# SaumikDana/Bayesian-Markov-chain-Monte-Carlo

Hardware: AMD Instinct MI355X
Metric: ode_steps_x_chains_per_sec (higher is better)
Workload: dtype f64

## Files before the change

### bayesian-markov-chain-monte-carlo_amd/csrc/rsf_device.h

```cpp
#pragma once
#include <hip/hip_runtime.h>
#include <stdint.h>

#include <type_traits>

#include "rsf_math.h"

namespace rsf {

struct Consts {
  double mu_ref, V_ref, k1, mu0;
  double a_def, b_def;
  double h, hh, h6;
  double inv_dt;
  double t0, dt;
  double inv_vref;
  double cacc;
  const double *vl;
  const double *data;
  int64_t group_chains;
  int32_t nout;
  int32_t S;
  int32_t kc;
  int32_t nchunks;
  double vl_lo, vl_hi;
};

__device__ __forceinline__ void select_group(Consts &K) {
  if (K.group_chains > 0) K.data += ((int64_t)blockIdx.x * blockDim.x / K.group_chains) * K.nout;
}

struct Lane {
  double inv_dc;
  double vdc;
  double kprime;
  double kia;
  double khh, kh, kh6;
  double vk;
  double beta;
  double kvk;
  double vrw;
  double hhdw, hdw;
  double cv;
  double h6v;
  double boa;
  double nhboa;
  double tc;
  double hhd, hd, h6d;
  double bh;
  double c_l1p, c_l1q;
  double c_em1;
  double cv2;
  double boa2;
  double bh2, bh4;
};

template <int T>
__device__ __forceinline__ void set_tier(Lane &L);

template <bool DAMP>
__device__ __forceinline__ Lane make_lane(double dc, double a, double b, const Consts &K) {
  Lane L;
  const double inv_a = fm::rcp(a);
  L.inv_dc = fm::rcp(dc);
  L.kprime = (1e-2 * 10) * L.inv_dc;
  L.kia = L.kprime * inv_a;
  L.khh = L.kia * K.hh;
  L.kh = L.kia * K.h;
  L.kh6 = L.kia * K.h6;
  const double via = K.V_ref * inv_a;
  L.vdc = K.V_ref * L.inv_dc;
  L.vk = via * L.kprime;
  L.beta = (b * K.V_ref) * (1.0 / (1e-2 * 10));
  L.kvk = K.k1 * via;
  const double ikw = DAMP ? fm::rcp(L.kvk) : 1.0;
  const double vkw = DAMP ? L.vk * ikw : L.vk;
  L.cv = K.cacc * vkw;
  L.h6v = K.h6 * vkw;
  L.boa = b * inv_a;
  L.tc = -K.mu_ref * inv_a;
  L.hhd = K.hh * L.vdc;
  L.hd = K.h * L.vdc;
  L.h6d = K.h6 * L.vdc;
  L.vrw = DAMP ? K.V_ref * ikw : K.V_ref;
  L.hhdw = DAMP ? L.hhd * ikw : L.hhd;
  L.hdw = DAMP ? L.hd * ikw : L.hd;
  L.nhboa = -0.5 * L.boa;
  L.bh = L.beta * fm::rcp(L.hhd);
  L.cv2 = 2.0 * L.cv;
  L.boa2 = 2.0 * L.boa;
  L.bh2 = -2.0 * L.bh;
  L.bh4 = 4.0 * L.bh;
  set_tier<2>(L);
  return L;
}


struct State {
  double ms, x, V;
  double w, rx;
};

template <bool DAMP>
__device__ __forceinline__ void rhs_tail(double w, double rx, double x, double vl, const Lane &L,
                                         const Consts &K, double &d0, double &d1, double &d2) {
  d1 = __builtin_fma(-w, x, 1.0);
  d0 = __builtin_fma(-K.V_ref, w, vl);
  const double bt = (L.beta * d1) * rx;
  double g = d0 - bt;
  if (DAMP) {
    const double kw = L.kvk * w;
    d0 = __builtin_fma(-kw, g, d0);
    g = d0 - bt;
    d2 = kw * g;
  } else {
    d2 = w * g;
  }
}

__device__ __forceinline__ void eval_full(double ms, double x, const Lane &L, const Consts &K, double &w, double &rx) {
  w = fm::exp(__builtin_fma(-L.boa, fm::log(x), __builtin_fma(ms, L.kia, L.tc)));
  rx = fm::rcp(x);
}

enum Tier : int { TIGHT = 0, NARROW = 1, WIDE = 2, FULL = 3 };

__device__ __forceinline__ double local_value(double x) {
  asm volatile("" : "+v"(x));
  return x;
}

template <bool DAMP, int T>
__device__ __forceinline__ void tier_enter(State &s, const Lane &L) {
  s.rx *= L.hhd;
  if (DAMP) s.w *= L.kvk;
}
template <int T>
__device__ __forceinline__ void tier_x(State &s, const Lane &L) { s.x = L.hhd * fm::rcp(s.rx); }
template <bool DAMP, int T>
__device__ __forceinline__ void tier_leave(State &s, const Lane &L) {
  tier_x<T>(s, L);
  s.rx *= fm::rcp(local_value(L.hhd));
  if (DAMP) s.w *= fm::rcp(local_value(L.kvk));
}
template <bool DAMP, int T>
__device__ __forceinline__ void eval_full_t(State &s, const Lane &L, const Consts &K) {
  eval_full(s.ms, s.x, L, K, s.w, s.rx);
  tier_enter<DAMP, T>(s, L);
}
template <bool DAMP, int T>
__device__ __forceinline__ void resync_t(State &s, const Lane &L, const Consts &K) {
  tier_x<T>(s, L);
  eval_full_t<DAMP, T>(s, L, K);
}


struct Guard {
  float rho, dlt;
  float dlt_h;
  float rho_f;
};

__device__ __forceinline__ float hi_as_float(double x) { return __builtin_bit_cast(float, __double2hiint(x)); }
constexpr float hi_pow2(int e) { return __builtin_bit_cast(float, (1023 + e) << 20); }


template <int T>
__device__ __forceinline__ void set_tier(Lane &L) {
  L.c_l1p = L.boa * (1.0 / 3.0);
  L.c_l1q = L.boa * (-1.0 / 4.0);
  L.c_em1 = T == TIGHT ? 1.0 / 24.0 : (T == NARROW ? 1.0 / 720.0 : 1.0 / 40320.0);
  asm volatile("" : "+v"(L.c_l1p), "+v"(L.c_l1q), "+v"(L.c_em1));
}

template <int T>
__device__ __forceinline__ bool guard_ok(const Guard &g) {
  return (g.rho < (T == WIDE ? hi_pow2(-11) : (T == NARROW ? hi_pow2(-14) : hi_pow2(-20)))) &&
         (g.dlt < (T == TIGHT ? hi_pow2(-9) : (T == NARROW ? hi_pow2(-7) : hi_pow2(-5)))) && (T != TIGHT || g.dlt_h < hi_pow2(-10));
}

constexpr float hi_pow2_34(int e) { return __builtin_bit_cast(float, ((1023 + e - 1) << 20) | 0x80000); }
template <int T>
__device__ __forceinline__ bool calm_enough(const Guard &g) {
  static_assert(T == NARROW || T == WIDE, "TIGHT has no tighter tier");
  return T == WIDE ? (g.rho < hi_pow2_34(-14) && g.dlt < hi_pow2_34(-7))
                   : (g.rho < hi_pow2_34(-20) && g.dlt < hi_pow2_34(-10));
}

constexpr int kResync = 512;

template <bool DAMP>
__device__ __forceinline__ double rk4_cold(State &s, double vl0, double vlm, double vl1, const Lane &L,
                                           const Consts &K) {
  double k0 = 0.0, k1 = 0.0, s0 = 0.0, s1 = 0.0, s2 = 0.0;
#pragma nounroll
  for (int st = 0; st < 4; ++st) {
    const double c = st == 0 ? 0.0 : (st == 3 ? K.h : K.hh);
    const double wgt = (st == 0 || st == 3) ? 1.0 : 2.0;
    const double vl = st == 0 ? vl0 : (st == 3 ? vl1 : vlm);
    const double x1 = __builtin_fma(c * L.vdc, k1, s.x);
    double w, rx, d0, d1, d2;
    eval_full(__builtin_fma(c, k0, s.ms), x1, L, K, w, rx);
    rhs_tail<DAMP>(w, rx, x1, vl, L, K, d0, d1, d2);
    s0 = __builtin_fma(wgt, d0, s0);
    s1 = __builtin_fma(wgt, d1, s1);
    s2 = __builtin_fma(wgt, d2, s2);
    k0 = d0;
    k1 = d1;
  }
  s.ms = __builtin_fma(K.h6, s0, s.ms);
  s.x = __builtin_fma(L.h6d, s1, s.x);
  return s2;
}

template <int T, bool HALF, bool SHORT = false, bool GUARD = true>
__device__ __forceinline__ void tight_incr(double rho, double dk, const Lane &L, double w0, double &w, double &q, Guard &g) {
  static_assert(!SHORT || (T == TIGHT && HALF), "the short series is for TIGHT's half-step stages");
  static_assert(GUARD || T == TIGHT, "only TIGHT has an a-priori bound");
  if constexpr (GUARD) g.rho = __builtin_fmaxf(g.rho, __builtin_fabsf(hi_as_float(rho)));
  double pb = L.nhboa;
  if (T == NARROW) pb = __builtin_fma(rho, L.c_l1p, pb);
  if (T == WIDE) pb = __builtin_fma(rho, __builtin_fma(rho, L.c_l1q, L.c_l1p), pb);
  const double dlt = __builtin_fma(-rho, __builtin_fma(rho, pb, L.boa), dk);
  if constexpr (GUARD) {
    if (T == TIGHT && HALF) g.dlt_h = __builtin_fmaxf(g.dlt_h, __builtin_fabsf(hi_as_float(dlt)));
    else g.dlt = __builtin_fmaxf(g.dlt, __builtin_fabsf(hi_as_float(dlt)));
  }
  double e = SHORT ? 1.0 / 6.0 : L.c_em1;
  if (T == WIDE) {
    e = fm::hfma(e, dlt, 1.0 / 5040.0);
    e = fm::hfma(e, dlt, 1.0 / 720.0);
  }
  if (T != TIGHT) {
    e = fm::hfma(e, dlt, 1.0 / 120.0);
    e = fm::hfma(e, dlt, 1.0 / 24.0);
  }
  if (!SHORT) e = fm::hfma(e, dlt, 1.0 / 6.0);
  e = __builtin_fma(e, dlt, 0.5);
  e = __builtin_fma(e, dlt, 1.0);
  w = __builtin_fma(w0 * dlt, e, w0);
  const double r1 = __builtin_fma(rho, rho, -rho);
  q = r1;
  if (T != TIGHT) q = __builtin_fma(-rho, q, -rho);
  if (T == WIDE) q = __builtin_fma(-rho, q, -rho);
}

template <bool GUARD = true>
__device__ __forceinline__ void tight_incr_doubled(double c1, double dk, const Lane &L, double w0, double &w, double &brx, Guard &g) {
  if constexpr (GUARD) g.rho_f = __builtin_fmaxf(g.rho_f, __builtin_fabsf(hi_as_float(c1)));
  const double dlt = __builtin_fma(-c1, __builtin_fma(-c1, L.boa2, L.boa2), dk);
  if constexpr (GUARD) g.dlt = __builtin_fmaxf(g.dlt, __builtin_fabsf(hi_as_float(dlt)));
  double e = fm::hfma(L.c_em1, dlt, 1.0 / 6.0);
  e = __builtin_fma(e, dlt, 0.5);
  e = __builtin_fma(e, dlt, 1.0);
  w = __builtin_fma(w0 * dlt, e, w0);
  brx = __builtin_fma(c1, __builtin_fma(c1, L.bh4, L.bh2), L.bh);
}

template <bool DAMP>
__device__ __forceinline__ void rhs_tight(double w, double xr, double Rh, double vl, double brx, double vr, double &d0, double &d1,
                                          double &g) {
  d1 = __builtin_fma(-w, xr, Rh);
  d0 = __builtin_fma(-vr, w, vl);
  g = __builtin_fma(-brx, d1, d0);
  if (DAMP) {
    d0 = __builtin_fma(-w, g, d0);
    g = __builtin_fma(-w, g, g);
  }
}

template <bool DAMP, int T, bool INSTEP = false, bool GUARD = true>
__device__ __forceinline__ double rk4_tight(State &s, double vl0, double vlm, double vl1, const Lane &L, const Consts &K, Guard &g,
                                            double obs = 0.0, double *ssq = nullptr, bool first = false) {
  static_assert(!INSTEP || T == TIGHT, "the in-step sum of squares is the TIGHT step's");
  static_assert(GUARD || INSTEP, "the unguarded step is the in-step mode's");
  double a0, a1, a2, b0, b1, b2, c0, c1, c2, e0, e1, e2, w, q;
  const double Rh = s.rx;
  const double vr = L.vrw, xh = L.hhdw, xf = L.hdw;
  rhs_tight<DAMP>(s.w, xh, Rh, vl0, L.bh, vr, a0, a1, a2);
  double sv = s.w * a2;
  tight_incr<T, true, INSTEP, GUARD>(a1, L.khh * a0, L, s.w, w, q, g);
  rhs_tight<DAMP>(w, __builtin_fma(xh, a1, xh), Rh, vlm, __builtin_fma(L.bh, q, L.bh), vr, b0, b1, b2);
  double sm = w * b2;
  tight_incr<T, true, INSTEP, GUARD>(b1, L.khh * b0, L, s.w, w, q, g);
  rhs_tight<DAMP>(w, __builtin_fma(xh, b1, xh), Rh, vlm, __builtin_fma(L.bh, q, L.bh), vr, c0, c1, c2);
  sm = __builtin_fma(w, c2, sm);
  if constexpr (INSTEP) {
    double brx;
    tight_incr_doubled<GUARD>(c1, L.kh * c0, L, s.w, w, brx, g);
    rhs_tight<DAMP>(w, __builtin_fma(xf, c1, xh), Rh, vl1, brx, vr, e0, e1, e2);
  } else {
    tight_incr<T, false>(c1 + c1, L.kh * c0, L, s.w, w, q, g);
    rhs_tight<DAMP>(w, __builtin_fma(xf, c1, xh), Rh, vl1, __builtin_fma(L.bh, q, L.bh), vr, e0, e1, e2);
  }
  sv = __builtin_fma(w, e2, sv);
  const double t0 = a0 + 2.0 * b0 + 2.0 * c0 + e0;
  const double t1 = a1 + 2.0 * b1 + 2.0 * c1 + e1;
  const double rho = t1 * (1.0 / 3.0);
  tight_incr<T, false, false, GUARD>(rho, L.kh6 * t0, L, s.w, w, q, g);
  s.ms = __builtin_fma(K.h6, t0, s.ms);
  s.w = w;
  s.rx = __builtin_fma(Rh, q, Rh);
  if constexpr (INSTEP) {
    const double r = __builtin_fma(sv, L.cv, __builtin_fma(sm, L.cv2, -obs));
    *ssq = first ? r * r : __builtin_fma(r, r, *ssq);
    return 0.0;
  }
  return __builtin_fma(2.0, sm, sv);
}

__device__ __forceinline__ State initial_state(double dc, const Lane &L, const Consts &K) {
  State s;
  s.ms = (K.mu0 * dc) * (1.0 / (1e-2 * 10));
  s.x = K.V_ref * ((dc * K.inv_vref) * L.inv_dc);
  s.V = K.V_ref;
  eval_full(s.ms, s.x, L, K, s.w, s.rx);
  return s;
}

constexpr int kLdsPad = 0;
__device__ __forceinline__ int lds_data_offset(const Consts &K) { return 2 * K.S * K.kc + 1 + kLdsPad; }
__device__ __forceinline__ int lds_d0_offset(const Consts &K) { return lds_data_offset(K) + K.kc; }

__device__ __forceinline__ void stage_chunk(double *lds, const Consts &K, int k0, int kn) {
  const int nv = 2 * K.S * kn + 1;
  const int base = 2 * K.S * (k0 - 1);
  __syncthreads();
  for (int i = threadIdx.x; i < nv; i += blockDim.x) lds[i] = K.vl[base + i];
  if (K.data) {
    double *ld = lds + lds_data_offset(K);
    for (int i = threadIdx.x; i < kn; i += blockDim.x) ld[i] = K.data[k0 + i];
    if (threadIdx.x == 0) lds[lds_d0_offset(K)] = K.data[0];
  }
  __syncthreads();
}

struct Emit {
  int ko;
  int phase;
  double vprev;
};

template <bool WANT_SSQ, bool WANT_ACC>
__device__ __forceinline__ void emit_at(double vnow, double vprev, int ko, double obs, const Consts &K, int k0,
                                        double &ssq, bool active, double *acc_out, int64_t stride) {
  const double ak = (vnow - vprev) * K.inv_dt;
  if (WANT_ACC && active) acc_out[(int64_t)(k0 + ko) * stride] = ak;
  if (WANT_SSQ) {
    const double r = ak - obs;
    ssq = __builtin_fma(r, r, ssq);
  }
}

template <bool WANT_SSQ, bool WANT_ACC>
__device__ __forceinline__ void emit_incr(double dvs, int ko, double obs, const Lane &L, int k0, double &ssq,
                                          bool active, double *acc_out, int64_t stride) {
  if (WANT_ACC && active) acc_out[(int64_t)(k0 + ko) * stride] = dvs * L.cv;
  if (WANT_SSQ) {
    const double r = __builtin_fma(dvs, L.cv, -obs);
    ssq = __builtin_fma(r, r, ssq);
  }
}

template <bool WANT_SSQ, bool WANT_ACC>
__device__ __forceinline__ void emit_sample(double vnow, Emit &em, double obs, const Consts &K, int k0, double &ssq,
                                            bool active, double *acc_out, int64_t stride) {
  emit_at<WANT_SSQ, WANT_ACC>(vnow, em.vprev, em.ko, obs, K, k0, ssq, active, acc_out, stride);
  em.vprev = vnow;
  ++em.ko;
}

template <bool DAMP, int T, int NU>
__device__ __forceinline__ bool trip_fast(const double *v, const Lane &L, const Consts &K, State &s, double (&dv)[NU], bool *calm = nullptr) {
  Guard g = {0, 0, 0, 0};
#pragma unroll
  for (int j = 0; j < NU; ++j) dv[j] = rk4_tight<DAMP, T>(s, v[2 * j], v[2 * j + 1], v[2 * j + 2], L, K, g);
  if constexpr (T != TIGHT) {
    if (calm) *calm = calm_enough<T>(g);
  }
  return !guard_ok<T>(g);
}

template <bool DAMP, int T, int NU>
__device__ __forceinline__ void trip_cold(const double *v, const Lane &L, const Consts &K, State &s, double (&dv)[NU]) {
  tier_x<T>(s, L);
#pragma unroll 1
  for (int j = 0; j < NU; ++j) {
    const double r = rk4_cold<DAMP>(s, v[2 * j], v[2 * j + 1], v[2 * j + 2], L, K);
#pragma unroll
    for (int m = 0; m < NU; ++m) dv[m] = m == j ? r : dv[m];
  }
  eval_full_t<DAMP, T>(s, L, K);
}

template <bool DAMP, int T, int NU>
__device__ __forceinline__ void trip_cold_ssq(const double *v, const double *ob, const Lane &L, const Consts &K, State &s, double &ssq) {
  tier_x<T>(s, L);
#pragma unroll 1
  for (int j = 0; j < NU; ++j) {
    const double dvs = rk4_cold<DAMP>(s, v[2 * j], v[2 * j + 1], v[2 * j + 2], L, K);
    emit_incr<true, false>(dvs, j, ob[j], L, 0, ssq, false, nullptr, 0);
  }
  eval_full_t<DAMP, T>(s, L, K);
}

template <bool DAMP, int NU>
__device__ __forceinline__ void trip_cold_plain(const double *v, const Lane &L, const Consts &K, State &s, double (&dv)[NU]) {
#pragma unroll 1
  for (int j = 0; j < NU; ++j) {
    const double r = rk4_cold<DAMP>(s, v[2 * j], v[2 * j + 1], v[2 * j + 2], L, K);
#pragma unroll
    for (int m = 0; m < NU; ++m) dv[m] = m == j ? r : dv[m];
  }
  eval_full(s.ms, s.x, L, K, s.w, s.rx);
}

constexpr int kFullRetry = 32;
constexpr int kCalmSteps = 16;
struct Wave {
  unsigned long long alive;
  unsigned long long need[3];
  unsigned long long stiff;
  int next_resync;
  int full_run;
  int calm;
  uint32_t steps[4], redone, lane_steps;
  double vl_lo, vl_hi;
  unsigned long long never;
  bool guard_next;
  uint32_t unguarded;
};

template <int NU>
struct TightBound {
  static constexpr double R = 0x1.0p-20, B = 0x1.0p-21, Dmax = 0.9 * 0x1.0p-9, gm1 = 1.02 * NU * Dmax;
  static constexpr double G = 1.02 * NU, kap = (NU + 1) * R, Bmax = 0.9 * B;
  static_assert(NU * Dmax < 0.035, "exp(x) - 1 <= 1.02 x needs x < 0.035");
};

__device__ __forceinline__ unsigned long long ballot(bool p) { return __builtin_amdgcn_ballot_w64(p); }
__device__ __forceinline__ bool lane_in(unsigned long long mask) { return (mask >> (threadIdx.x & 63)) & 1; }
template <int CTRL>
__device__ __forceinline__ double dpp_move(double v) {
  const int lo = __builtin_amdgcn_update_dpp(0, __double2loint(v), CTRL, 0xF, 0xF, false);
  const int hi = __builtin_amdgcn_update_dpp(0, __double2hiint(v), CTRL, 0xF, 0xF, false);
  return __hiloint2double(hi, lo);
}

template <int NU>
__device__ __forceinline__ void wave_begin(Wave &W, bool active, const Lane &L, const Consts &K) {
  const double dk = 1.2 * K.V_ref * K.h * L.kia;
  using TB = TightBound<NU>;
  const double dmin = __builtin_fma(__builtin_fabs(L.kh), 0.5 * (K.vl_hi - K.vl_lo), __builtin_fabs(L.boa) * TB::R);
  const double rmin = __builtin_fabs(L.hhd) * __builtin_fma(dmin, TB::G, TB::kap);
  W.never = ballot(active && !(dmin < TB::Dmax && rmin < TB::Bmax));
  W.guard_next = false;
  W.alive = ballot(active);
  W.need[0] = ballot(active && !(dk < 0x1.0p-9));
  W.need[1] = ballot(active && !(dk < 0x1.0p-7));
  W.need[2] = W.stiff = ballot(active && !(dk < 0x1.0p-3));
  W.next_resync = kResync;
  W.full_run = 0;
  W.calm = 0;
  W.vl_lo = K.vl_lo;
  W.vl_hi = K.vl_hi;
  asm volatile("" : "+s"(W.vl_lo), "+s"(W.vl_hi));
}

__device__ __forceinline__ int wave_tier(const Wave &W) {
  return (W.need[2] & W.alive) ? FULL : ((W.need[1] & W.alive) ? WIDE : ((W.need[0] & W.alive) ? NARROW : TIGHT));
}

template <bool DAMP, int NU, bool GUARD = true>
__device__ __forceinline__ unsigned long long trip_fast_ssq(const double *v, const double (&obs)[NU], const Lane &L, const Consts &K, State &s,
                                                            double &tsum) {
  Guard g = {0, 0, 0, 0};
#pragma unroll
  for (int j = 0; j < NU; ++j) rk4_tight<DAMP, TIGHT, true, GUARD>(s, v[2 * j], v[2 * j + 1], v[2 * j + 2], L, K, g, obs[j], &tsum, j == 0);
  if constexpr (!GUARD) return 0ull;
  return ballot(!(g.rho < hi_pow2(-20))) | ballot(!(g.rho_f < hi_pow2(-21))) | ballot(!(g.dlt < hi_pow2(-9))) | ballot(!(g.dlt_h < hi_pow2(-10)));
}

template <bool DAMP, int NU>
__device__ __forceinline__ unsigned long long tight_needs_guard(const State &s, const Lane &L, const Wave &W) {
  using TB = TightBound<NU>;
  constexpr double R = TB::R, B = TB::B, Dmax = TB::Dmax, gm1 = TB::gm1;
  const double p = L.vrw * s.w;
  const double c = __builtin_fma(-s.w, L.hhdw, s.rx);
  double D0 = __builtin_fma(__builtin_fabs(p), gm1, __builtin_fmax(__builtin_fabs(W.vl_hi - p), __builtin_fabs(W.vl_lo - p)));
  if (DAMP) D0 = __builtin_fma((1.0 + gm1) * __builtin_fabs(s.w), __builtin_fma(__builtin_fabs(L.bh), B, D0), D0);
  const double D = __builtin_fma(__builtin_fabs(L.kh), D0, __builtin_fabs(L.boa) * R);
  const double rb = __builtin_fma(__builtin_fabs(s.rx) + __builtin_fabs(c), __builtin_fma(D, TB::G, TB::kap), __builtin_fabs(c));
  return ballot(!(D < Dmax)) | ballot(!(rb < TB::Bmax));
}

template <bool WANT_SSQ, bool WANT_ACC, bool S1, int NU>
__device__ __forceinline__ void emit_trip(const double (&dv)[NU], const double (&obs)[NU], const double *ld, int r, State &s, Emit &em,
                                          const Lane &L, const Consts &K, int k0, double &ssq, bool active, double *acc_out, int64_t stride) {
  if (S1) {
#pragma unroll
    for (int j = 0; j < NU; ++j) emit_incr<WANT_SSQ, WANT_ACC>(dv[j], r + j, obs[j], L, k0, ssq, active, acc_out, stride);
  } else {
#pragma unroll
    for (int j = 0; j < NU; ++j) {
      s.V = __builtin_fma(L.h6v, dv[j], s.V);
      if (++em.phase == K.S) {
        em.phase = 0;
        const double o = WANT_SSQ ? ld[em.ko] : 0.0;
        emit_sample<WANT_SSQ, WANT_ACC>(s.V, em, o, K, k0, ssq, active, acc_out, stride);
      }
    }
  }
}

constexpr int kTightUnroll = 8;
constexpr int kNarrowUnroll = 8, kWiderUnroll = 4;
template <bool DAMP, bool WANT_SSQ, bool WANT_ACC, int T, bool S1, int NU, bool INSTEP = false, bool UNGUARD = false>
__device__ __forceinline__ int integrate_multi(const double *lds, const double *ld, const Consts &K, Lane L, int k0, int kn, int r,
                                               int nsteps, State &s, Emit &em, double &ssq, double thr, bool active, double *acc_out,
                                               int64_t stride, Wave &W) {
  static_assert(NU >= 1 && (kResync % NU) == 0, "trip lengths divide the resync interval");
  static_assert(!INSTEP || (T == TIGHT && WANT_SSQ && !WANT_ACC && S1), "the in-step sum of squares: TIGHT, SSq alone, one step per sample");
  static_assert(!UNGUARD || (INSTEP && NU > 2), "whole trips of the in-step mode; the remainder's pairs keep the guard");
  constexpr bool HELD = INSTEP && NU > 2 && !UNGUARD;
  set_tier<T>(L);
  const bool held = HELD && (W.never & W.alive) != 0;
  for (; r + NU <= nsteps; r += NU) {
    const unsigned long long deadmask = WANT_SSQ ? ballot(ssq > thr) : 0ull;
    const double *v = lds + 2 * r;
    double obs[NU], dv[INSTEP ? 1 : NU];
#pragma unroll
    for (int j = 0; j < NU; ++j) obs[j] = (WANT_SSQ && S1) ? ld[r + j] : 0.0;
    if (r >= W.next_resync) {
      resync_t<DAMP, T>(s, L, K);
      W.next_resync = (r & ~(kResync - 1)) + kResync;
    }
    if constexpr (UNGUARD) {
      if ((tight_needs_guard<DAMP, NU>(s, L, W) & W.alive) != 0) {
        W.guard_next = true;
        return r;
      }
      double usum = 0.0;
      trip_fast_ssq<DAMP, NU, false>(v, obs, L, K, s, usum);
      W.steps[T] += NU;
      W.unguarded += NU;
      W.lane_steps += NU * (uint32_t)__builtin_popcountll(W.alive);
      ssq += usum;
      W.alive &= ~deadmask;
      if (W.alive == 0) return r + NU;
    } else {
    const State save = s;
    bool calm = false;
    double tsum = 0.0;
    unsigned long long tripped;
    if constexpr (INSTEP) tripped = trip_fast_ssq<DAMP, NU>(v, obs, L, K, s, tsum);
    else tripped = ballot(trip_fast<DAMP, T, NU>(v, L, K, s, dv, &calm));
    const unsigned long long badmask = tripped & W.alive;
    W.steps[T] += NU;
    W.lane_steps += NU * (uint32_t)__builtin_popcountll(W.alive);
    if constexpr (T != TIGHT) {
      W.calm = (ballot(!calm) & W.alive) == 0 ? W.calm + NU : 0;
    }
    if (__builtin_expect(badmask != 0, 0)) {
      if (lane_in(badmask)) {
        s = save;
        if constexpr (INSTEP) {
          tsum = 0.0;
          trip_cold_ssq<DAMP, T, NU>(v, ld + r, L, K, s, ssq);
        } else {
          trip_cold<DAMP, T, NU>(v, L, K, s, dv);
        }
      }
      W.need[T] |= badmask;
      W.redone += NU;
      W.full_run = 0;
      W.calm = 0;
    }
    if constexpr (INSTEP) ssq += tsum;
    else emit_trip<WANT_SSQ, WANT_ACC, S1, NU>(dv, obs, ld, r, s, em, L, K, k0, ssq, active, acc_out, stride);
    const bool died = HELD && (deadmask & W.alive) != 0;
    W.alive &= ~deadmask;
    if constexpr (T != TIGHT) {
      if (W.calm >= kCalmSteps && badmask == 0) {
        W.need[T - 1] &= ~W.alive | W.stiff;
        W.calm = 0;
      }
    }
    if (badmask != 0 || W.alive == 0 || (T != TIGHT && (W.need[T - 1] & W.alive) == 0)) return r + NU;
    if constexpr (HELD) {
      if (!held || (died && (W.never & W.alive) == 0)) return r + NU;
    }
    }
  }
  return r;
}

template <bool DAMP, bool WANT_SSQ, bool WANT_ACC, bool S1>
__device__ __forceinline__ int integrate_full(const double *lds, const double *ld, const Consts &K, const Lane &L, int k0, int kn, int r,
                                              int nsteps, State &s, Emit &em, double &ssq, double thr, bool active, double *acc_out,
                                              int64_t stride, Wave &W) {
#pragma unroll 1
  for (; r < nsteps; ++r) {
    const unsigned long long deadmask = WANT_SSQ ? ballot(ssq > thr) : 0ull;
    const double *v = lds + 2 * r;
    const double obs[1] = {(WANT_SSQ && S1) ? ld[r] : 0.0};
    const double dv[1] = {rk4_cold<DAMP>(s, v[0], v[1], v[2], L, K)};
    W.steps[FULL] += 1;
    W.lane_steps += (uint32_t)__builtin_popcountll(W.alive);
    emit_trip<WANT_SSQ, WANT_ACC, S1, 1>(dv, obs, ld, r, s, em, L, K, k0, ssq, active, acc_out, stride);
    W.alive &= ~deadmask;
    if (++W.full_run >= kFullRetry) {
      W.need[2] &= W.stiff;
      W.full_run = 0;
    }
    if (W.alive == 0 || (W.need[2] & W.alive) == 0) return r + 1;
  }
  return r;
}

__device__ __forceinline__ int start_tier(const Lane &L, const Consts &K) {
  const double dk = 1.2 * K.V_ref * K.h * L.kia;
  return !__any(!(dk < 0x1.0p-9)) ? TIGHT : (!__any(!(dk < 0x1.0p-7)) ? NARROW : WIDE);
}

constexpr int kLockstepTrip = 8;
template <bool DAMP, typename OnSample, typename AfterTrip>
__device__ __forceinline__ void integrate_lockstep(double *lds, const Consts &K, const Lane &L, State &st, int kn, OnSample on_sample,
                                                   AfterTrip after_trip) {
  constexpr int NU = kLockstepTrip;
  static_assert(kResync % NU == 0, "the resync test looks at the first step of a trip");
  const int nsteps = K.S * kn;
  double dsum = 0.0;
  int phase = 0, ko = 0;
  int tier = start_tier(L, K);
  int r = 0;
  auto trip = [&](auto tier_tag, auto nu_tag) {
    constexpr int T = decltype(tier_tag)::value, NUT = decltype(nu_tag)::value;
    const double *v = lds + 2 * r;
    Lane Lt = L;
    set_tier<T>(Lt);
    const State save = st;
    double dv[NUT];
    tier_enter<DAMP, T>(st, Lt);
    const bool bad = trip_fast<DAMP, T, NUT>(v, Lt, K, st, dv);
    tier_leave<DAMP, T>(st, Lt);
    const bool any_bad = ballot(bad) != 0;
    if (__builtin_expect(any_bad, 0)) {
      if (bad) {
        st = save;
        trip_cold_plain<DAMP, NUT>(v, L, K, st, dv);
      }
    }
#pragma unroll
    for (int j = 0; j < NUT; ++j) {
      dsum += dv[j];
      if (++phase == K.S) {
        phase = 0;
        on_sample(dsum * L.cv, ko);
        dsum = 0.0;
        ++ko;
      }
    }
    return any_bad;
  };
  for (; r + NU <= nsteps; r += NU) {
    if ((r & (kResync - 1)) == 0) eval_full(st.ms, st.x, L, K, st.w, st.rx);
    bool any_bad;
    if (tier == TIGHT) any_bad = trip(std::integral_constant<int, TIGHT>{}, std::integral_constant<int, NU>{});
    else if (tier == NARROW) any_bad = trip(std::integral_constant<int, NARROW>{}, std::integral_constant<int, NU>{});
    else any_bad = trip(std::integral_constant<int, WIDE>{}, std::integral_constant<int, NU>{});
    if (any_bad && tier < WIDE) ++tier;
    after_trip();
  }
  for (; r < nsteps; ++r) {
    if ((r & (kResync - 1)) == 0) eval_full(st.ms, st.x, L, K, st.w, st.rx);
    trip(std::integral_constant<int, WIDE>{}, std::integral_constant<int, 1>{});
    after_trip();
  }
}

template <bool DAMP, bool WANT_SSQ, bool WANT_ACC, int T, bool S1, int NU, bool INSTEP = false>
__device__ __forceinline__ int integrate_tier(const double *lds, const double *ld, const Consts &K, const Lane &L, int k0, int kn, int r,
                                              int nsteps, State &s, Emit &em, double &ssq, double thr, bool active, double *acc_out,
                                              int64_t stride, Wave &W) {
  if (r + NU <= nsteps) {
    if constexpr (INSTEP) {
      if ((W.never & W.alive) == 0 && !W.guard_next) return integrate_multi<DAMP, WANT_SSQ, WANT_ACC, T, S1, NU, true, true>(lds, ld, K, L, k0, kn, r, nsteps, s, em, ssq, thr, active, acc_out, stride, W);
    }
    W.guard_next = false;
    return integrate_multi<DAMP, WANT_SSQ, WANT_ACC, T, S1, NU, INSTEP>(lds, ld, K, L, k0, kn, r, nsteps, s, em, ssq, thr, active, acc_out, stride, W);
  }
  return integrate_multi<DAMP, WANT_SSQ, WANT_ACC, T, S1, 2, INSTEP>(lds, ld, K, L, k0, kn, r, nsteps, s, em, ssq, thr, active, acc_out, stride, W);
}

template <bool DAMP, bool WANT_SSQ, bool WANT_ACC, bool S1, int NUT, bool SSQ_IN_STEP>
__device__ __forceinline__ void integrate_tiers(const double *lds, const double *ld, const Consts &K, const Lane &L, int k0,
                                                int kn, State &s, double &ssq, double thr, bool active, double *acc_out, int64_t stride, Wave &W) {
  constexpr bool INSTEP = SSQ_IN_STEP && WANT_SSQ && !WANT_ACC && S1;
  const int nsteps = S1 ? kn : K.S * kn;
  Emit em = {0, 0, s.V};
  int r = 0;
  W.next_resync = kResync;
  bool scaled = false;
  while (r < nsteps && W.alive != 0) {
    const int tier = wave_tier(W);
    if (tier == FULL) {
      if (scaled) { tier_leave<DAMP, WIDE>(s, L); scaled = false; }
      r = integrate_full<DAMP, WANT_SSQ, WANT_ACC, S1>(lds, ld, K, L, k0, kn, r, nsteps, s, em, ssq, thr, active, acc_out, stride, W);
      eval_full(s.ms, s.x, L, K, s.w, s.rx);
      continue;
    }
    if (!scaled) { tier_enter<DAMP, TIGHT>(s, L); scaled = true; }
    if (nsteps - r == 1) r = integrate_multi<DAMP, WANT_SSQ, WANT_ACC, WIDE, S1, 1>(lds, ld, K, L, k0, kn, r, nsteps, s, em, ssq, thr, active, acc_out, stride, W);
    else if (tier == TIGHT) r = integrate_tier<DAMP, WANT_SSQ, WANT_ACC, TIGHT, S1, NUT, INSTEP>(lds, ld, K, L, k0, kn, r, nsteps, s, em, ssq, thr, active, acc_out, stride, W);
    else if (tier == NARROW) r = integrate_tier<DAMP, WANT_SSQ, WANT_ACC, NARROW, S1, kNarrowUnroll>(lds, ld, K, L, k0, kn, r, nsteps, s, em, ssq, thr, active, acc_out, stride, W);
    else r = integrate_tier<DAMP, WANT_SSQ, WANT_ACC, WIDE, S1, kWiderUnroll>(lds, ld, K, L, k0, kn, r, nsteps, s, em, ssq, thr, active, acc_out, stride, W);
  }
  if (scaled) tier_leave<DAMP, WIDE>(s, L);
}

template <bool DAMP, bool WANT_SSQ, bool WANT_ACC, int NUT, bool SSQ_IN_STEP>
__device__ __forceinline__ void integrate_chunk(const double *lds, const Consts &K, const Lane &L, int k0, int kn, State &s,
                                                double &ssq, double thr, bool active, double *acc_out, int64_t stride, Wave &W) {
  const double *ld = lds + lds_data_offset(K);
  if (K.S == 1) integrate_tiers<DAMP, WANT_SSQ, WANT_ACC, true, NUT, SSQ_IN_STEP>(lds, ld, K, L, k0, kn, s, ssq, thr, active, acc_out, stride, W);
  else integrate_tiers<DAMP, WANT_SSQ, WANT_ACC, false, NUT, SSQ_IN_STEP>(lds, ld, K, L, k0, kn, s, ssq, thr, active, acc_out, stride, W);
}

template <bool DAMP, bool WANT_SSQ, bool WANT_ACC, int NUT = kTightUnroll, bool SSQ_IN_STEP = false>
__device__ __forceinline__ double solve(double *lds, const Consts &K, bool resident, bool active, double dc, double a,
                                        double b, double thr, double *acc_out, int64_t stride, Wave &W) {
  const Lane L = make_lane<DAMP>(dc, a, b, K);
  State s = initial_state(dc, L, K);
  wave_begin<NUT>(W, active, L, K);
  double ssq = 0.0;
  if (WANT_ACC && active) acc_out[0] = 0.0;
  for (int k0 = 1; k0 < K.nout; k0 += K.kc) {
    const int kn = min(K.kc, K.nout - k0);
    if (!resident) stage_chunk(lds, K, k0, kn);
    if (WANT_SSQ && k0 == 1) {
      const double d0 = lds[lds_d0_offset(K)];
      ssq = d0 * d0;
    }
    if (W.alive != 0) integrate_chunk<DAMP, WANT_SSQ, WANT_ACC, NUT, SSQ_IN_STEP>(lds, K, L, k0, kn, s, ssq, thr, active, acc_out, stride, W);
  }
  return ssq;
}

enum : uint32_t { SLOT_Z01 = 0, SLOT_Z2 = 1, SLOT_U = 2, SLOT_GAMMA = 8 };

__device__ __forceinline__ void philox4x32_10(uint32_t c0, uint32_t c1, uint32_t c2, uint32_t c3, uint32_t k0,
                                              uint32_t k1, uint32_t out[4]) {
#pragma unroll
  for (int r = 0; r < 10; ++r) {
    const uint32_t hi0 = __umulhi(0xD2511F53u, c0), lo0 = 0xD2511F53u * c0;
    const uint32_t hi1 = __umulhi(0xCD9E8D57u, c2), lo1 = 0xCD9E8D57u * c2;
    const uint32_t n0 = hi1 ^ c1 ^ k0, n2 = hi0 ^ c3 ^ k1;
    c0 = n0; c1 = lo1; c2 = n2; c3 = lo0;
    k0 += 0x9E3779B9u;
    k1 += 0xBB67AE85u;
  }
  out[0] = c0; out[1] = c1; out[2] = c2; out[3] = c3;
}

__device__ __forceinline__ void draw_words(uint64_t seed, uint64_t chain, uint32_t iter, uint32_t slot,
                                           uint32_t w[4]) {
  philox4x32_10((uint32_t)chain, (uint32_t)(chain >> 32), iter, slot, (uint32_t)seed, (uint32_t)(seed >> 32), w);
}

__device__ __forceinline__ double u53(uint32_t hi, uint32_t lo) {
  const uint64_t k = (((uint64_t)hi << 32) | lo) >> 11;
  return (double)(k + 1) * 0x1.0p-53;
}

__device__ __forceinline__ void normal_pair(const uint32_t w[4], double &z0, double &z1) {
  const double u1 = u53(w[0], w[1]), u2 = u53(w[2], w[3]);
  const double r = sqrt(-2.0 * fm::log(u1));
  double s, c;
  fm::sincos2pi(u2, s, c);
  z0 = r * c;
  z1 = r * s;
}

__device__ __forceinline__ double rng_log(double x) { return fm::log(x); }

__device__ __forceinline__ double gamma_draw(uint64_t seed, uint64_t chain, uint32_t iter, double d, double c) {
  for (uint32_t j = 0; j < 64; ++j) {
    uint32_t w[4];
    double x, unused;
    draw_words(seed, chain, iter, SLOT_GAMMA + 2 * j, w);
    normal_pair(w, x, unused);
    double v = 1.0 + c * x;
    if (!(v > 0.0)) continue;
    v = v * v * v;
    draw_words(seed, chain, iter, SLOT_GAMMA + 2 * j + 1, w);
    const double u = u53(w[0], w[1]);
    if (rng_log(u) < 0.5 * x * x + d * (1.0 - v + rng_log(v))) return d * v;
  }
  return d;
}

template <int D>
__device__ __forceinline__ bool chol_lower(const double *V, double *L) {
  bool ok = true;
#pragma unroll
  for (int e = 0; e < D * D; ++e) L[e] = 0.0;
#pragma unroll
  for (int j = 0; j < D; ++j) {
    double s = V[j * D + j];
#pragma unroll
    for (int k = 0; k < j; ++k) s -= L[j * D + k] * L[j * D + k];
    if (!(s > 0.0)) { ok = false; continue; }
    const double ljj = sqrt(s);
    L[j * D + j] = ljj;
#pragma unroll
    for (int i = j + 1; i < D; ++i) {
      double t = V[i * D + j];
#pragma unroll
      for (int k = 0; k < j; ++k) t -= L[i * D + k] * L[j * D + k];
      L[i * D + j] = t / ljj;
    }
  }
  return ok;
}

template <int D>
__device__ __forceinline__ void sym_inverse(const double *A, double *Ai) {
  if (D == 1) {
    Ai[0] = 1.0 / A[0];
  } else {
    const double c00 = A[4] * A[8] - A[5] * A[7], c01 = A[5] * A[6] - A[3] * A[8], c02 = A[3] * A[7] - A[4] * A[6];
    const double id = 1.0 / (A[0] * c00 + A[1] * c01 + A[2] * c02);
    Ai[0] = c00 * id; Ai[1] = (A[2] * A[7] - A[1] * A[8]) * id; Ai[2] = (A[1] * A[5] - A[2] * A[4]) * id;
    Ai[3] = c01 * id; Ai[4] = (A[0] * A[8] - A[2] * A[6]) * id; Ai[5] = (A[2] * A[3] - A[0] * A[5]) * id;
    Ai[6] = c02 * id; Ai[7] = (A[1] * A[6] - A[0] * A[7]) * id; Ai[8] = (A[0] * A[4] - A[1] * A[3]) * id;
  }
}

template <int D>
__device__ __forceinline__ bool window_covariance(const double *ws, const double *wq, double nn, double scale, const double *eps, double *Vn,
                                                  double *Ln) {
#pragma unroll
  for (int p = 0; p < D; ++p)
#pragma unroll
    for (int r = 0; r < D; ++r) Vn[p * D + r] = scale * ((wq[p * D + r] - ws[p] * ws[r] / nn) / (nn - 1.0) + (p == r ? eps[p] : 0.0));
  return chol_lower<D>(Vn, Ln);
}

template <typename F>
__device__ __forceinline__ double np_cov_1d(F a, int n) {
  double sum;
  if (n < 8) {
    sum = 0.0;
    for (int i = 0; i < n; ++i) sum += a(i);
  } else {
    double r[8];
#pragma unroll
    for (int j = 0; j < 8; ++j) r[j] = a(j);
    int i = 8;
    for (; i < n - (n % 8); i += 8)
#pragma unroll
      for (int j = 0; j < 8; ++j) r[j] += a(i + j);
    sum = ((r[0] + r[1]) + (r[2] + r[3])) + ((r[4] + r[5]) + (r[6] + r[7]));
    for (; i < n; ++i) sum += a(i);
  }
  const double avg = sum / (double)n;
  double c = 0.0;
  for (int k = 0; k < n; ++k) {
    const double dlt = a(k) - avg;
    c = __builtin_fma(dlt, dlt, c);
  }
  return c * (1.0 / (double)(n - 1));
}

}
```

Baseline: 389.5 billion.

## Rescale TIGHT in-step increments with per-lane series coefficients and pairwise guard folding

Replaces the TIGHT in-step exponential-increment math with a per-stage scaled form (tight_incr_scaled) whose series coefficients are precomputed once per integrate call in a Series struct. This removes the per-stage multiply by khh/kh/kh6 and folds those constants into the polynomial. The guard now uses lane-dependent limits and folds maxima over pairs of steps to cut fmax work. Observations are loaded only a few steps ahead rather than all up front, to reduce register pressure. In exchange it adds registers for the Series coefficients, and the guard thresholds change semantics.

After: 397.3 billion (median of 6 runs). +2.0%, better.

```diff
diff --git a/bayesian-markov-chain-monte-carlo_amd/csrc/rsf_device.h b/bayesian-markov-chain-monte-carlo_amd/csrc/rsf_device.h
--- a/bayesian-markov-chain-monte-carlo_amd/csrc/rsf_device.h
+++ b/bayesian-markov-chain-monte-carlo_amd/csrc/rsf_device.h
@@ -51,7 +51,6 @@
   double c_l1p, c_l1q;
   double c_em1;
   double cv2;
-  double boa2;
   double bh2, bh4;
 };
 
@@ -88,7 +87,6 @@
   L.nhboa = -0.5 * L.boa;
   L.bh = L.beta * fm::rcp(L.hhd);
   L.cv2 = 2.0 * L.cv;
-  L.boa2 = 2.0 * L.boa;
   L.bh2 = -2.0 * L.bh;
   L.bh4 = 4.0 * L.bh;
   set_tier<2>(L);
@@ -159,6 +157,9 @@
   float rho, dlt;
   float dlt_h;
   float rho_f;
+  float del;
+  float del_e;
+  float p_rho, p_rho_f, p_del, p_del_e;
 };
 
 __device__ __forceinline__ float hi_as_float(double x) { return __builtin_bit_cast(float, __double2hiint(x)); }
@@ -213,20 +214,16 @@
   return s2;
 }
 
-template <int T, bool HALF, bool SHORT = false, bool GUARD = true>
+template <int T, bool HALF>
 __device__ __forceinline__ void tight_incr(double rho, double dk, const Lane &L, double w0, double &w, double &q, Guard &g) {
-  static_assert(!SHORT || (T == TIGHT && HALF), "the short series is for TIGHT's half-step stages");
-  static_assert(GUARD || T == TIGHT, "only TIGHT has an a-priori bound");
-  if constexpr (GUARD) g.rho = __builtin_fmaxf(g.rho, __builtin_fabsf(hi_as_float(rho)));
+  g.rho = __builtin_fmaxf(g.rho, __builtin_fabsf(hi_as_float(rho)));
   double pb = L.nhboa;
   if (T == NARROW) pb = __builtin_fma(rho, L.c_l1p, pb);
   if (T == WIDE) pb = __builtin_fma(rho, __builtin_fma(rho, L.c_l1q, L.c_l1p), pb);
   const double dlt = __builtin_fma(-rho, __builtin_fma(rho, pb, L.boa), dk);
-  if constexpr (GUARD) {
-    if (T == TIGHT && HALF) g.dlt_h = __builtin_fmaxf(g.dlt_h, __builtin_fabsf(hi_as_float(dlt)));
-    else g.dlt = __builtin_fmaxf(g.dlt, __builtin_fabsf(hi_as_float(dlt)));
-  }
-  double e = SHORT ? 1.0 / 6.0 : L.c_em1;
+  if (T == TIGHT && HALF) g.dlt_h = __builtin_fmaxf(g.dlt_h, __builtin_fabsf(hi_as_float(dlt)));
+  else g.dlt = __builtin_fmaxf(g.dlt, __builtin_fabsf(hi_as_float(dlt)));
+  double e = L.c_em1;
   if (T == WIDE) {
     e = fm::hfma(e, dlt, 1.0 / 5040.0);
     e = fm::hfma(e, dlt, 1.0 / 720.0);
@@ -235,7 +232,7 @@
     e = fm::hfma(e, dlt, 1.0 / 120.0);
     e = fm::hfma(e, dlt, 1.0 / 24.0);
   }
-  if (!SHORT) e = fm::hfma(e, dlt, 1.0 / 6.0);
+  e = fm::hfma(e, dlt, 1.0 / 6.0);
   e = __builtin_fma(e, dlt, 0.5);
   e = __builtin_fma(e, dlt, 1.0);
   w = __builtin_fma(w0 * dlt, e, w0);
@@ -245,16 +242,74 @@
   if (T == WIDE) q = __builtin_fma(-rho, q, -rho);
 }
 
-template <bool GUARD = true>
-__device__ __forceinline__ void tight_incr_doubled(double c1, double dk, const Lane &L, double w0, double &w, double &brx, Guard &g) {
-  if constexpr (GUARD) g.rho_f = __builtin_fmaxf(g.rho_f, __builtin_fabsf(hi_as_float(c1)));
-  const double dlt = __builtin_fma(-c1, __builtin_fma(-c1, L.boa2, L.boa2), dk);
-  if constexpr (GUARD) g.dlt = __builtin_fmaxf(g.dlt, __builtin_fabsf(hi_as_float(dlt)));
-  double e = fm::hfma(L.c_em1, dlt, 1.0 / 6.0);
-  e = __builtin_fma(e, dlt, 0.5);
-  e = __builtin_fma(e, dlt, 1.0);
-  w = __builtin_fma(w0 * dlt, e, w0);
-  brx = __builtin_fma(c1, __builtin_fma(c1, L.bh4, L.bh2), L.bh);
+struct Series {
+  double B, N, N6;
+  double h1, h2;
+  double f1, f2, f3;
+  double e1, e2, e3;
+  float lim, lim_e;
+};
+template <bool GUARD>
+__device__ __forceinline__ Series make_series(const Lane &L) {
+  Series S;
+  const double khh = local_value(L.khh);
+  const double ik = fm::rcp(khh);
+  S.B = L.boa * ik;
+  S.N = -0.5 * S.B;
+  S.N6 = S.B * (-1.0 / 6.0);
+  const double kh = khh + khh, kh6 = khh * (1.0 / 3.0);
+  const double k2 = khh * khh, f2 = kh * kh, e2 = kh6 * kh6;
+  S.h1 = 0.5 * k2;
+  S.h2 = (k2 * khh) * (1.0 / 6.0);
+  S.f1 = 0.5 * f2;
+  S.f2 = (f2 * kh) * (1.0 / 6.0);
+  S.f3 = (f2 * f2) * (1.0 / 24.0);
+  S.e1 = 0.5 * e2;
+  S.e2 = (e2 * kh6) * (1.0 / 6.0);
+  S.e3 = (e2 * e2) * (1.0 / 24.0);
+  S.lim = S.lim_e = 0.0f;
+  if constexpr (GUARD) {
+    const double aik = (1.0 - 0x1.0p-30) * __builtin_fabs(ik);
+    S.lim = hi_as_float(0x1.0p-10 * aik);
+    S.lim_e = hi_as_float(0x1.8p-8 * aik);
+  }
+  return S;
+}
+
+__device__ __forceinline__ void guard_note(float &acc, float &pend, double x, bool odd) {
+  const float ax = __builtin_fabsf(hi_as_float(x));
+  if (odd) acc = __builtin_fmaxf(__builtin_fmaxf(acc, pend), ax);
+  else pend = ax;
+}
+
+template <int STAGE, bool GUARD>
+__device__ __forceinline__ void tight_incr_scaled(double r, double d, const Lane &L, const Series &S, double w0, double &w, double &q, Guard &g,
+                                                  bool odd) {
+  const double pb = STAGE == 0 ? __builtin_fma(r, S.N, S.B) : (STAGE == 1 ? __builtin_fma(-r, S.B, S.B) : __builtin_fma(r, S.N6, S.B));
+  const double del = __builtin_fma(-r, pb, d);
+  double e;
+  if constexpr (STAGE == 0) e = __builtin_fma(__builtin_fma(S.h2, del, S.h1), del, L.khh);
+  else if constexpr (STAGE == 1) e = __builtin_fma(__builtin_fma(fm::hfma(S.f3, del, S.f2), del, S.f1), del, L.kh);
+  else e = __builtin_fma(__builtin_fma(fm::hfma(S.e3, del, S.e2), del, S.e1), del, L.kh6);
+  w = __builtin_fma(w0 * del, e, w0);
+  if constexpr (STAGE == 1) {
+    q = __builtin_fma(r, __builtin_fma(r, L.bh4, L.bh2), L.bh);
+    if constexpr (GUARD) {
+      guard_note(g.rho_f, g.p_rho_f, r, odd);
+      guard_note(g.del, g.p_del, del, odd);
+    }
+  } else {
+    const double rho = STAGE == 0 ? r : r * (1.0 / 3.0);
+    q = __builtin_fma(rho, rho, -rho);
+    if constexpr (GUARD && STAGE == 0) {
+      g.rho = __builtin_fmaxf(g.rho, __builtin_fabsf(hi_as_float(rho)));
+      g.del = __builtin_fmaxf(g.del, __builtin_fabsf(hi_as_float(del)));
+    }
+    if constexpr (GUARD && STAGE == 2) {
+      guard_note(g.rho, g.p_rho, rho, odd);
+      guard_note(g.del_e, g.p_del_e, del, odd);
+    }
+  }
 }
 
 template <bool DAMP>
@@ -271,7 +326,8 @@
 
 template <bool DAMP, int T, bool INSTEP = false, bool GUARD = true>
 __device__ __forceinline__ double rk4_tight(State &s, double vl0, double vlm, double vl1, const Lane &L, const Consts &K, Guard &g,
-                                            double obs = 0.0, double *ssq = nullptr, bool first = false) {
+                                            double obs = 0.0, double *ssq = nullptr, bool first = false, const Series *S = nullptr,
+                                            bool odd = false) {
   static_assert(!INSTEP || T == TIGHT, "the in-step sum of squares is the TIGHT step's");
   static_assert(GUARD || INSTEP, "the unguarded step is the in-step mode's");
   double a0, a1, a2, b0, b1, b2, c0, c1, c2, e0, e1, e2, w, q;
@@ -279,15 +335,17 @@
   const double vr = L.vrw, xh = L.hhdw, xf = L.hdw;
   rhs_tight<DAMP>(s.w, xh, Rh, vl0, L.bh, vr, a0, a1, a2);
   double sv = s.w * a2;
-  tight_incr<T, true, INSTEP, GUARD>(a1, L.khh * a0, L, s.w, w, q, g);
+  if constexpr (INSTEP) tight_incr_scaled<0, GUARD>(a1, a0, L, *S, s.w, w, q, g, odd);
+  else tight_incr<T, true>(a1, L.khh * a0, L, s.w, w, q, g);
   rhs_tight<DAMP>(w, __builtin_fma(xh, a1, xh), Rh, vlm, __builtin_fma(L.bh, q, L.bh), vr, b0, b1, b2);
   double sm = w * b2;
-  tight_incr<T, true, INSTEP, GUARD>(b1, L.khh * b0, L, s.w, w, q, g);
+  if constexpr (INSTEP) tight_incr_scaled<0, GUARD>(b1, b0, L, *S, s.w, w, q, g, odd);
+  else tight_incr<T, true>(b1, L.khh * b0, L, s.w, w, q, g);
   rhs_tight<DAMP>(w, __builtin_fma(xh, b1, xh), Rh, vlm, __builtin_fma(L.bh, q, L.bh), vr, c0, c1, c2);
   sm = __builtin_fma(w, c2, sm);
   if constexpr (INSTEP) {
     double brx;
-    tight_incr_doubled<GUARD>(c1, L.kh * c0, L, s.w, w, brx, g);
+    tight_incr_scaled<1, GUARD>(c1, c0, L, *S, s.w, w, brx, g, odd);
     rhs_tight<DAMP>(w, __builtin_fma(xf, c1, xh), Rh, vl1, brx, vr, e0, e1, e2);
   } else {
     tight_incr<T, false>(c1 + c1, L.kh * c0, L, s.w, w, q, g);
@@ -296,8 +354,12 @@
   sv = __builtin_fma(w, e2, sv);
   const double t0 = a0 + 2.0 * b0 + 2.0 * c0 + e0;
   const double t1 = a1 + 2.0 * b1 + 2.0 * c1 + e1;
-  const double rho = t1 * (1.0 / 3.0);
-  tight_incr<T, false, false, GUARD>(rho, L.kh6 * t0, L, s.w, w, q, g);
+  if constexpr (INSTEP) {
+    tight_incr_scaled<2, GUARD>(t1, t0, L, *S, s.w, w, q, g, odd);
+  } else {
+    const double rho = t1 * (1.0 / 3.0);
+    tight_incr<T, false>(rho, L.kh6 * t0, L, s.w, w, q, g);
+  }
   s.ms = __builtin_fma(K.h6, t0, s.ms);
   s.w = w;
   s.rx = __builtin_fma(Rh, q, Rh);
@@ -471,14 +533,30 @@
   return (W.need[2] & W.alive) ? FULL : ((W.need[1] & W.alive) ? WIDE : ((W.need[0] & W.alive) ? NARROW : TIGHT));
 }
 
+template <int NU>
+constexpr int kObsAhead = NU < 4 ? NU : 4;
 template <bool DAMP, int NU, bool GUARD = true>
-__device__ __forceinline__ unsigned long long trip_fast_ssq(const double *v, const double (&obs)[NU], const Lane &L, const Consts &K, State &s,
-                                                            double &tsum) {
-  Guard g = {0, 0, 0, 0};
-#pragma unroll
-  for (int j = 0; j < NU; ++j) rk4_tight<DAMP, TIGHT, true, GUARD>(s, v[2 * j], v[2 * j + 1], v[2 * j + 2], L, K, g, obs[j], &tsum, j == 0);
+__device__ __forceinline__ unsigned long long trip_fast_ssq(const double *v, const double (&head)[kObsAhead<NU>], const double *ob, const Lane &L,
+                                                            const Series &S, const Consts &K, State &s, double &tsum) {
+  static_assert(NU % 2 == 0, "the guard folds the figures of two steps (guard_note); observations come in pairs");
+  constexpr int AH = kObsAhead<NU>;
+  Guard g = {};
+  double obs[NU];
+#pragma unroll
+  for (int j = 0; j < AH; ++j) obs[j] = head[j];
+#pragma unroll
+  for (int j = 0; j < NU; ++j) {
+    if (j % 2 == 0 && j + AH < NU) {
+      obs[j + AH] = ob[j + AH];
+      obs[j + AH + 1] = ob[j + AH + 1];
+    }
+    rk4_tight<DAMP, TIGHT, true, GUARD>(s, v[2 * j], v[2 * j + 1], v[2 * j + 2], L, K, g, obs[j], &tsum, j == 0, &S, (j & 1) != 0);
+    if constexpr (GUARD) {
+      if (j & 1) asm volatile("" : "+v"(g.rho), "+v"(g.rho_f), "+v"(g.del), "+v"(g.del_e));
+    }
+  }
   if constexpr (!GUARD) return 0ull;
-  return ballot(!(g.rho < hi_pow2(-20))) | ballot(!(g.rho_f < hi_pow2(-21))) | ballot(!(g.dlt < hi_pow2(-9))) | ballot(!(g.dlt_h < hi_pow2(-10)));
+  return ballot(!(g.rho < hi_pow2(-20))) | ballot(!(g.rho_f < hi_pow2(-21))) | ballot(!(g.del < S.lim)) | ballot(!(g.del_e < S.lim_e));
 }
 
 template <bool DAMP, int NU>
@@ -524,13 +602,16 @@
   static_assert(!UNGUARD || (INSTEP && NU > 2), "whole trips of the in-step mode; the remainder's pairs keep the guard");
   constexpr bool HELD = INSTEP && NU > 2 && !UNGUARD;
   set_tier<T>(L);
+  Series S;
+  if constexpr (INSTEP) S = make_series<!UNGUARD>(L);
   const bool held = HELD && (W.never & W.alive) != 0;
   for (; r + NU <= nsteps; r += NU) {
     const unsigned long long deadmask = WANT_SSQ ? ballot(ssq > thr) : 0ull;
     const double *v = lds + 2 * r;
-    double obs[NU], dv[INSTEP ? 1 : NU];
-#pragma unroll
-    for (int j = 0; j < NU; ++j) obs[j] = (WANT_SSQ && S1) ? ld[r + j] : 0.0;
+    constexpr int NOBS = INSTEP ? kObsAhead<NU> : NU;
+    double obs[NOBS], dv[INSTEP ? 1 : NU];
+#pragma unroll
+    for (int j = 0; j < NOBS; ++j) obs[j] = (WANT_SSQ && S1) ? ld[r + j] : 0.0;
     if (r >= W.next_resync) {
       resync_t<DAMP, T>(s, L, K);
       W.next_resync = (r & ~(kResync - 1)) + kResync;
@@ -541,7 +622,7 @@
         return r;
       }
       double usum = 0.0;
-      trip_fast_ssq<DAMP, NU, false>(v, obs, L, K, s, usum);
+      trip_fast_ssq<DAMP, NU, false>(v, obs, ld + r, L, S, K, s, usum);
       W.steps[T] += NU;
       W.unguarded += NU;
       W.lane_steps += NU * (uint32_t)__builtin_popcountll(W.alive);
@@ -553,7 +634,7 @@
     bool calm = false;
     double tsum = 0.0;
     unsigned long long tripped;
-    if constexpr (INSTEP) tripped = trip_fast_ssq<DAMP, NU>(v, obs, L, K, s, tsum);
+    if constexpr (INSTEP) tripped = trip_fast_ssq<DAMP, NU>(v, obs, ld + r, L, S, K, s, tsum);
     else tripped = ballot(trip_fast<DAMP, T, NU>(v, L, K, s, dv, &calm));
     const unsigned long long badmask = tripped & W.alive;
     W.steps[T] += NU;
```
